# NeRdTheNed/deft4j

Hardware: AMD Instinct MI355X
Metric: input MB/s on raw-deflate optimise (mode NONE) (higher is better)
Workload: dtype u8

## Files before the change

### deft4j_amd/__init__.py

```python
import ctypes
import os

_HERE = os.path.dirname(os.path.abspath(__file__))
LIB_PATH = os.path.join(_HERE, "libdeft4g.so")

_lib = None
_ready = False


class d4g_stats(ctypes.Structure):
    _fields_ = [(n, ctypes.c_double) for n in ("ms_upload", "ms_parse", "ms_optimise", "ms_merge", "ms_write", "ms_total")] + \
               [(n, ctypes.c_int64) for n in ("n_streams", "n_blocks", "n_tokens", "bytes_in", "bytes_decoded", "bytes_out",
                                              "rounds", "kernel_launches", "search_bytes_algorithmic")] + \
               [("ms_search_kernels", ctypes.c_double), ("ms_parse_kernels", ctypes.c_double)] + \
               [(n, ctypes.c_int64) for n in ("scan_candidates", "scan_confirmed", "exact_probes", "jump_rounds")] + \
               [("ms_state_kernels", ctypes.c_double), ("state_launches", ctypes.c_int64), ("state_tokens_per_round", ctypes.c_int64),
                ("state_bytes_per_round", ctypes.c_int64), ("search_lanes", ctypes.c_int64), ("ms_checksum_kernels", ctypes.c_double),
                ("ms_lz_sort", ctypes.c_double), ("ms_lz_parse", ctypes.c_double), ("ms_lz_emit", ctypes.c_double),
                ("lz_parse_passes", ctypes.c_int64), ("lz_chunks_rerun", ctypes.c_int64), ("lz_symbols", ctypes.c_int64),
                ("ms_recompress_encode", ctypes.c_double), ("ms_recompress_encode_front", ctypes.c_double),
                ("ms_recompress_encode_search", ctypes.c_double), ("ms_recompress_reoptimise", ctypes.c_double),
                ("recompress_outputs", ctypes.c_int64), ("recompress_outputs_pruned", ctypes.c_int64),
                ("ms_zopfli_table", ctypes.c_double), ("ms_zopfli_split", ctypes.c_double), ("ms_zopfli_squeeze", ctypes.c_double),
                ("ms_zopfli_emit", ctypes.c_double), ("zopfli_blocks", ctypes.c_int64), ("zopfli_position_iterations", ctypes.c_int64),
# ... 50 lines not shown
VERIFY_OK, VERIFY_SKIPPED, VERIFY_PARSE, VERIFY_SIZE, VERIFY_LENGTH, VERIFY_BYTES = 0, 1, -1, -2, -3, -4
VERDICT_NAMES = {0: "OK", 1: "SKIPPED", -1: "PARSE", -2: "SIZE", -3: "LENGTH", -4: "BYTES"}
BLOCK_TYPE_NAMES = ("STORED", "FIXED", "DYNAMIC")

ENC_JVM, ENC_JZLIB = 0, 1
STRATEGY_DEFAULT, STRATEGY_FILTERED, STRATEGY_HUFFMAN_ONLY = 0, 1, 2
STRATEGY_RLE, STRATEGY_FIXED = 3, 4

EXPORTS = ["d4g_init", "d4g_shutdown", "d4g_last_error", "d4g_batch_create", "d4g_batch_run", "d4g_batch_stream_result",
           "d4g_batch_copy_output", "d4g_batch_copy_decoded", "d4g_batch_checksums", "d4g_batch_parse", "d4g_batch_stats", "d4g_batch_destroy", "d4g_optimise_streams",
           "d4g_size_bits_fallback", "d4g_inflate", "d4g_free", "d4g_batch_create_encode", "d4g_batch_run_encode", "d4g_deflate_streams",
           "d4g_compress", "d4g_recompress_streams", "d4g_batch_run_recompress", "d4g_batch_recompress_result", "d4g_zopfli_streams",
           "d4g_debug_zopfli_table", "d4g_debug_zopfli_code_lengths", "d4g_debug_cl_tree_lengths", "d4g_init_devices", "d4g_device_count", "d4g_set_device",
           "d4g_batch_create_on", "d4g_optimise_streams_sharded", "d4g_batch_create_encode_level", "d4g_deflate_streams_level",
           "d4g_batch_verify", "d4g_batch_verify_result", "d4g_verify_streams", "d4g_debug_batch_poke_output", "d4g_batch_block_info", "d4g_debug_verify_compare",
           "d4g_debug_device_blocks", "d4g_batch_parse_error", "d4g_diagnose_streams", "d4g_parse_reason_name",
           "d4g_find_streams", "d4g_batch_recover", "d4g_batch_copy_recovered", "d4g_recover_streams"]


def load_library(path=None):
    global _lib
    if _lib is not None and path is None:
        return _lib
    p = path or os.environ.get("D4G_LIB") or LIB_PATH
    if not os.path.exists(p):
        raise RuntimeError("libdeft4g.so is not built (%s): run `python -c 'import __graft_entry__ as g; g.build()'`; "
                           "there is no CPU fallback" % p)
    L = ctypes.CDLL(p)
    L.d4g_init.restype = ctypes.c_int
    L.d4g_init.argtypes = [ctypes.c_int]
    L.d4g_shutdown.restype = None
# ... 76 lines not shown
    L.d4g_optimise_streams_sharded.restype = ctypes.c_int
    L.d4g_optimise_streams_sharded.argtypes = L.d4g_optimise_streams.argtypes
    L.d4g_batch_verify.restype = ctypes.c_int
    L.d4g_batch_verify.argtypes = [ctypes.c_void_p]
    L.d4g_batch_verify_result.restype = ctypes.c_int
    L.d4g_batch_verify_result.argtypes = [ctypes.c_void_p, ctypes.c_size_t, ctypes.POINTER(ctypes.c_int32), ctypes.POINTER(ctypes.c_int64)]
    L.d4g_verify_streams.restype = ctypes.c_int
    L.d4g_verify_streams.argtypes = [ctypes.c_size_t, ctypes.POINTER(ctypes.c_char_p), ctypes.POINTER(ctypes.c_size_t), ctypes.POINTER(ctypes.c_char_p),
                                     ctypes.POINTER(ctypes.c_size_t), ctypes.POINTER(ctypes.c_int32), ctypes.POINTER(ctypes.c_int64)]
    L.d4g_debug_batch_poke_output.restype = ctypes.c_int
    L.d4g_debug_batch_poke_output.argtypes = [ctypes.c_void_p, ctypes.c_size_t, ctypes.c_size_t, ctypes.c_uint8]
    L.d4g_debug_verify_compare.restype = ctypes.c_int
    L.d4g_debug_verify_compare.argtypes = [ctypes.c_char_p, ctypes.c_size_t, ctypes.c_char_p, ctypes.c_size_t, ctypes.c_size_t, ctypes.POINTER(ctypes.c_int64)]
    L.d4g_debug_device_blocks.restype = ctypes.c_int
    L.d4g_debug_device_blocks.argtypes = [ctypes.POINTER(ctypes.c_int64)]
    L.d4g_batch_block_info.restype = ctypes.c_int
    L.d4g_batch_block_info.argtypes = [ctypes.c_void_p, ctypes.c_size_t, ctypes.c_int, ctypes.POINTER(d4g_block_info), ctypes.c_size_t,
                                       ctypes.POINTER(ctypes.c_size_t)]
    L.d4g_batch_parse_error.restype = ctypes.c_int
    L.d4g_batch_parse_error.argtypes = [ctypes.c_void_p, ctypes.c_size_t, ctypes.POINTER(d4g_parse_error)]
    L.d4g_diagnose_streams.restype = ctypes.c_int
    L.d4g_diagnose_streams.argtypes = [ctypes.c_size_t, ctypes.POINTER(ctypes.c_char_p), ctypes.POINTER(ctypes.c_size_t), ctypes.POINTER(d4g_parse_error)]
    L.d4g_parse_reason_name.restype = ctypes.c_char_p
    L.d4g_parse_reason_name.argtypes = [ctypes.c_int]
    L.d4g_find_streams.restype = ctypes.c_int
    L.d4g_find_streams.argtypes = [ctypes.c_size_t, ctypes.POINTER(ctypes.c_char_p), ctypes.POINTER(ctypes.c_size_t), ctypes.POINTER(d4g_find_options),
                                   ctypes.POINTER(ctypes.POINTER(d4g_found_stream)), ctypes.POINTER(ctypes.c_size_t), ctypes.POINTER(d4g_find_stats)]
    L.d4g_batch_recover.restype = ctypes.c_int
    L.d4g_batch_recover.argtypes = [ctypes.c_void_p]
    L.d4g_batch_copy_recovered.restype = ctypes.c_int
# ... 548 lines not shown
```

### deft4j_amd/csrc/d4g_arch.h

```cpp
#pragma once
#include <stdint.h>

#ifndef D4G_HOSTSIM
#include <hip/hip_runtime.h>
#endif

#if defined(D4G_PROFILE_OPS) && defined(D4G_HOSTSIM)
#error "D4G_PROFILE_OPS counts GPU clock cycles: the emulator build has no clock"
#endif

#define D4G_DEV __device__ __forceinline__

#if defined(D4G_HOSTSIM) && !defined(D4G_SIM_WAVE_HEAP)
#define D4G_SERIAL_TREES
#endif

#ifdef D4G_HOSTSIM
#define D4G_SIM_LOG(...) fprintf(stderr, __VA_ARGS__)
#else
#define D4G_SIM_LOG(...) ((void)0)
#endif

#define D4G_BASE_PRIO 1
#ifdef D4G_HOSTSIM
// ... 37 lines not shown
#endif
}

D4G_DEV int wave_sum_i32(int v) {
#ifdef D4G_HOSTSIM
    for (int m = 32; m >= 1; m >>= 1) v = (int)((unsigned)v + (unsigned)__shfl_xor(v, m));
    return v;
#else
    v += __builtin_amdgcn_update_dpp(0, v, 0x111, 0xf, 0xf, false);
    v += __builtin_amdgcn_update_dpp(0, v, 0x112, 0xf, 0xf, false);
    v += __builtin_amdgcn_update_dpp(0, v, 0x114, 0xf, 0xf, false);
    v += __builtin_amdgcn_update_dpp(0, v, 0x118, 0xf, 0xf, false);
    v += __builtin_amdgcn_update_dpp(0, v, 0x142, 0xa, 0xf, false);
    v += __builtin_amdgcn_update_dpp(0, v, 0x143, 0xc, 0xf, false);
    return __builtin_amdgcn_readlane(v, 63);
#endif
}

D4G_DEV uint32_t wave_min_u32(uint32_t v) {
#ifdef D4G_HOSTSIM
    for (int m = 32; m >= 1; m >>= 1) { const uint32_t o = __shfl_xor(v, m); v = o < v ? o : v; }
    return v;
#else
    int x = (int)v;
    auto step = [&](int o) { x = (int)((uint32_t)o < (uint32_t)x ? (uint32_t)o : (uint32_t)x); };
    step(__builtin_amdgcn_update_dpp(-1, x, 0x111, 0xf, 0xf, false));
    step(__builtin_amdgcn_update_dpp(-1, x, 0x112, 0xf, 0xf, false));
    step(__builtin_amdgcn_update_dpp(-1, x, 0x114, 0xf, 0xf, false));
    step(__builtin_amdgcn_update_dpp(-1, x, 0x118, 0xf, 0xf, false));
    step(__builtin_amdgcn_update_dpp(-1, x, 0x142, 0xa, 0xf, false));
// ... 95 lines not shown
```

### deft4j_amd/csrc/d4g_host.h

```cpp
#pragma once
#include <algorithm>
#include <chrono>
#include <cstring>
#include <map>
#include <memory>
#include <atomic>
#include <vector>

#include "d4g_ops.h"
#include "d4g_fused.h"
#include "d4g_parse.h"
#include "d4g_rt.h"
#include "d4g_write.h"
#include "d4g_knobs.h"
#include "d4g_program.h"
#include "../../include/deft4g.h"

namespace d4g {

#define D4G_SEG_TARGET_BYTES 8192
#define D4G_SEG_MAX_BYTES (1LL << 20)
#define D4G_SEG_MAX_TOKENS (1LL << 16)
static inline int seg_threads() {
#ifdef D4G_HOSTSIM
    return parse_threads();
#else
    return 1024;
#endif
}

static inline double now_ms() {
    return std::chrono::duration<double, std::milli>(std::chrono::steady_clock::now().time_since_epoch()).count();
}

struct HBlock {
    int type = 0;
    int gpu = -1;
    int homeGpu = -1;
    int ordinal = 0;
    i64 tokStart = 0, tokCount = 0, uStart = 0, uLen = 0;
    i64 refStart = 0, refCount = 0;
    i64 size = 0;
// ... 188 lines not shown
```

### deft4j_amd/csrc/d4g_host_parse.h

```cpp
#pragma once

namespace d4g {

inline void Batch::create(size_t n, const uint8_t* const* in, const size_t* len, bool fromDevice) {
    memset(&stats, 0, sizeof(stats));
    double t0 = now_ms();
    streams.resize(n);
    i64 off = 0;
    for (size_t i = 0; i < n; i++) {
        streams[i].inOff = off;
        streams[i].inLen = (i64)len[i];
        off += ((i64)len[i] + 15) & ~15LL;
        off += 16;
        stats.bytes_in += (i64)len[i];
    }
    i64 total = off + D4G_INCH + 64;
    dIn.alloc_zero((size_t)total);
    for (size_t i = 0; i < n; i++) {
        if (fromDevice) rt_d2d(dIn + streams[i].inOff, in[i], len[i]);
        else rt_h2d(dIn + streams[i].inOff, in[i], len[i]);
    }
    rt_sync();
    stats.n_streams = (i64)n;
    stats.ms_upload = now_ms() - t0;
// ... 485 lines not shown
            R.maxSlots = std::max(R.maxSlots, (i64)(segs.size() - first) - 1);
            for (size_t q = first; q < segs.size(); q++)
                for (i64 o = 0; o < segs[q].uLen; o += D4G_SUB_CHUNK)
                    R.chunks.push_back({si, segs[q].win, segs[q].uStart + o, std::min<i64>(D4G_SUB_CHUNK, segs[q].uLen - o)});
        }
        i = j;
    }
    return R;
}
inline void Batch::copy_block_local(const std::vector<D4GTokRange>& allRanges, const CopyRoute& R, int32_t* dBad, RtScratch& tmp) {
    D4GTokRange* dAll = tmp.upload(allRanges);
    D4GSegment* dSegs = tmp.upload(R.segs);
    uint16_t* dSym = tmp.alloc<uint16_t>((size_t)uTotal, 64);
    const size_t slots = R.slotOrd.size();
    uint16_t* dTailA = slots ? tmp.alloc<uint16_t>(slots * D4G_WIN) : nullptr;
    RT_LAUNCH(k_seg_symbols, R.segs.size(), seg_threads(), dStreams, dSegs, dAll, dTok, dU, dSym, dTailA, dBad);
    stats.kernel_launches++;
    stats.copy_segments += (i64)R.segs.size();
    if (R.maxSlots > 1) {
        int32_t* dOrd = tmp.upload(R.slotOrd);
        uint16_t* dTailB = tmp.alloc<uint16_t>(slots * D4G_WIN);
        const int GC = 4;
        for (i64 d = 1; d < R.maxSlots; d <<= 1) {
            RT_LAUNCH(k_seg_compose, slots * GC, 256, dOrd, dTailA, dTailB, (int)d, GC);
            std::swap(dTailA, dTailB);
            stats.kernel_launches++;
            stats.copy_rounds++;
        }
    }
    if (!R.chunks.empty()) {
        D4GSubChunk* dChunks = tmp.upload(R.chunks);
// ... 78 lines not shown
        }
        bool done = false;
        for (int k = 0; k < JB; k++) {
            stats.jump_rounds++;
            if (ch[k] < stopNum) { done = true; break; }
        }
        if (done) break;
    }
    RT_LAUNCH(k_resolve_streams, n * (size_t)G, 256, dStreamsD, dSrc, dU, G);
    stats.kernel_launches++;
}
inline void Batch::block_bins(const std::vector<int32_t>& realBlocks, bool needSlots, RtScratch& tmp) {
    if (!needSlots || realBlocks.empty()) return;
    int32_t* dReal = tmp.upload(realBlocks);
    D4GCtx c = make_ctx(engine().progDyn, 0);
    RT_LAUNCH(k_block_bins, realBlocks.size() * D4G_BINS_SPLIT, 256, c, dReal);
    stats.kernel_launches++;
}

}
```

### deft4j_amd/csrc/d4g_host_write.h

```cpp
#pragma once

namespace d4g {

inline void Batch::phase_write() {
    std::vector<D4GWriteJob> jobs;
    i64 words = 0;
    for (HStream& s : streams) {
        s.outWordBase = words;
        if (s.status != 0) continue;
        i64 pos = 0;
        for (size_t k = 0; k < s.blocks.size(); k++) {
            const HBlock& b = s.blocks[k];
            D4GWriteJob j;
            memset(&j, 0, sizeof(j));
            j.blk = b.gpu;
            j.type = b.type;
            j.isFinal = k + 1 == s.blocks.size();
            j.bitStart = words * 32 + pos;
            j.uAbs = s.uBase + b.uStart;
            j.uLen = b.uLen;
            jobs.push_back(j);
            pos += 3;
            pos += b.size_at(pos);
        }
// ... 73 lines not shown
    phase_write();
    double t4 = now_ms();
    stats.ms_parse = t1 - t0;
    stats.ms_optimise = t2 - t1b;
    stats.ms_merge = t3 - t2;
    stats.ms_write = t4 - t3;
    stats.ms_total = (t1 - t0) + (t4 - t1b);
    stats.ms_search_kernels = msSearch;
    stats.ms_parse_kernels = msParseKernels;
    stats.search_bytes_algorithmic = stats.bytes_in + stats.bytes_decoded + stats.bytes_out;
    release_scratch();
}
inline void Batch::release_scratch() {
    rt_sync_all();
    dTok.reset(); dRefs.reset(); dTokRef.reset();
    dBinStat.reset(); dBinMask.reset();
    dHsMemo.reset(); dRcMemo.reset(); dPassMemo.reset();
    dBlocks.reset(); dStates.reset(); dMasks.reset();
    dKeys.reset(); dActive.reset(); dResults.reset();
    dReady.reset(); dHeads.reset();
}

enum { VERIFY_OK = 0, VERIFY_SKIPPED = 1, VERIFY_PARSE = -1, VERIFY_SIZE = -2, VERIFY_LENGTH = -3, VERIFY_BYTES = -4 };
struct VerifyItem {
    const uint8_t* bytes = nullptr;
    size_t len = 0;
    const uint8_t* want = nullptr;
    i64 wantLen = 0;
    i64 wantBits = -1;
    int verdict = VERIFY_SKIPPED;
    i64 first = -1;
// ... 63 lines not shown
```

### deft4j_amd/csrc/d4g_knobs.h

```cpp
#pragma once
#include <algorithm>
#include <cstdlib>
#include <cstring>
#include <stdexcept>

#include "d4g_ops.h"
#include "d4g_fused.h"
#include "d4g_rt.h"

namespace d4g {

static inline const char* knob_now(const char* name) { return getenv(name); }
static inline int knob_now(const char* name, int def) { const char* t = getenv(name); return t ? atoi(t) : def; }
static inline long long knob_now_ll(const char* name, long long def) { const char* t = getenv(name); return t ? atoll(t) : def; }
#define KNOB_ONCE(name, def) ([] { static const int v = knob_now(name, def); return v; }())
static inline bool knob_is_zero(const char* t) { return t && t[0] == '0'; }

static inline bool exec_fused() { const char* t = knob_now("D4G_EXEC"); return !t || !strcmp(t, "fused"); }
static inline int exec_persistent(int nActive = 0) {
    const char* t = knob_now("D4G_EXEC");
    const int mode = !t ? 2 : !strcmp(t, "levels") ? 0 : !strcmp(t, "persistent") ? 1 : 2;
    const int maxBlocks = knob_now("D4G_PERSIST_MAX_BLOCKS", 128);
#ifdef D4G_HOSTSIM
    return mode == 0 ? 0 : 1;
// ... 56 lines not shown
#endif
    return v == 128 || v == 256 || v == 512 ? v : 64;
}
enum { D4G_COPY_AUTO = 0, D4G_COPY_DOUBLING = 1, D4G_COPY_BLOCKS = 2 };
static inline int copy_mode() {
    const char* t = knob_now("D4G_COPY");
    if (!t || !strcmp(t, "auto")) return D4G_COPY_AUTO;
    if (!strcmp(t, "doubling")) return D4G_COPY_DOUBLING;
    if (!strcmp(t, "blocks")) return D4G_COPY_BLOCKS;
    throw std::runtime_error("D4G_COPY must be doubling, blocks or auto");
}
static inline int jump_stop_pct() { return KNOB_ONCE("D4G_JUMP_STOP_PCT", 50); }
static inline int jump_tile_reps() { return KNOB_ONCE("D4G_JUMP_TILE_REPS", 6); }
static inline int jump_threads() { return KNOB_ONCE("D4G_JUMP_THREADS", 1024); }
static inline int jump_lds_kb() { return KNOB_ONCE("D4G_JUMP_LDS_KB", 70); }

static inline bool verify_switch() { const char* v = knob_now("D4G_VERIFY"); return v && v[0] && !(v[0] == '0' && !v[1]); }
static inline void pool_max_bytes(size_t* bytes) { if (const char* t = knob_now("D4G_POOL_MAX_MB")) *bytes = (size_t)atoll(t) << 20; }
static inline long long group_blocks() { return knob_now("D4G_GROUP_BLOCKS", 12000); }
static inline bool zf_table_scan() { const char* t = knob_now("D4G_ZF_TABLE"); return t && !strcmp(t, "scan"); }
static inline int zf_pool_words() { const char* t = knob_now("D4G_ZF_POOL_WORDS"); return t ? std::max(64, atoi(t)) : 0; }

static inline bool debug_rounds() { return knob_now("D4G_DEBUG_ROUNDS") != nullptr; }
static inline bool debug_jump() { return knob_now("D4G_DEBUG_JUMP") != nullptr; }
static inline int debug_program() { const char* t = knob_now("D4G_DEBUG_PROGRAM"); return !t ? 0 : atoi(t) >= 2 ? 2 : 1; }
static inline int debug_zopfli() { return knob_now("D4G_DEBUG_ZOPFLI", 0); }

}
```

### deft4j_amd/csrc/d4g_ops.h

```cpp
#pragma once
#include "d4g_device.h"

#ifdef D4G_PROFILE_OPS
__device__ unsigned long long d4g_dbg_pass[4];
__device__ unsigned long long d4g_dbg_hdr[4];
#endif

#ifndef D4G_HSMEMO_SLOTS
#define D4G_HSMEMO_SLOTS 64
#endif
struct D4GHsMemo {
    unsigned long long tag;
    unsigned long long check;
    int32_t state;
    int32_t hdr;
    int32_t lane;
    int32_t nLit;
    int32_t n, pad;
    uint32_t key[(D4G_NLIT + D4G_NDIST) / 4];
};

#ifndef D4G_RCMEMO_SLOTS
#define D4G_RCMEMO_SLOTS 128
#endif
// ... 379 lines not shown
        atomicAdd(&d4g_dbg_pass[3], (unsigned long long)nRef);
    }
#endif
    if (mine) {
        for (int i = threadIdx.x; i < D4G_HIST; i += blockDim.x) d4g_st_agent((uint32_t*)&mine->delta[i], (uint32_t)((int)S->hist[i] - histBefore[i]));
        if (threadIdx.x == 0) {
            d4g_st_agent((uint64_t*)&mine->saved, (uint64_t)saved);
            d4g_st_agent((uint64_t*)&mine->check, (uint64_t)h2);
        }
        d4g_drain_stores();
        __syncthreads();
        if (threadIdx.x == 0) d4g_st_agent(&mine->state, 2);
    }
}

#define D4G_BINS_SPLIT 4
__global__ void __launch_bounds__(256) k_block_bins(D4GCtx c, const int32_t* blockList) {
    __shared__ uint32_t T[D4G_NBINS * D4G_BINSTRIDE];
    const D4GBlock b = c.blocks[blockList[blockIdx.x / D4G_BINS_SPLIT]];
    const int part = blockIdx.x % D4G_BINS_SPLIT;
    if (b.binStat < 0) return;
    for (int i = threadIdx.x; i < D4G_NBINS * D4G_BINSTRIDE; i += blockDim.x) T[i] = 0;
    __syncthreads();
    const uint4* rf = c.refs + b.refStart;
    const uint8_t* Ub = c.U + b.uBase;
    uint64_t* bm = c.binMask + b.binMask;
    const int lane = threadIdx.x & 63;
    const int nRef = (int)b.refCount, nWords = (int)b.maskWords;
    for (int r0 = part * (int)blockDim.x; r0 < nWords * 64; r0 += D4G_BINS_SPLIT * (int)blockDim.x) {
        int r = r0 + threadIdx.x;
        uint4 rv = r < nRef ? rf[r] : make_uint4(0u, 0u, 0u, 0u);
        int len = ref_len(rv.x);
        int bin = ref_lsym(rv.x) - 257;
        if (len > 0) {
            const uint32_t* uw = (const uint32_t*)Ub + (rv.y >> 2);
            const int sh = (int)(rv.y & 3u) * 8;
            uint32_t w0 = uw[0], w1 = uw[1], w2 = uw[2];
            c.refs[b.refStart + r].z = d4g_alignbit(w1, w0, sh);
            c.refs[b.refStart + r].w = d4g_alignbit(w2, w1, sh);
            uint32_t* row = T + bin * D4G_BINSTRIDE;
            atomicAdd(&row[D4G_BIN_DIST + ref_dsym(rv.x)], 1u);
            atomicAdd(&row[D4G_BIN_COUNT], 1u);
            atomicAdd(&row[D4G_BIN_EBITS], (unsigned)ref_ebits(rv.x));
            for_bytes(Ub + rv.y, len, [&](int by) { atomicAdd(&row[by], 1u); return true; });
        }
        unsigned long long todo = d4g_ballot(len > 0);
        while (todo) {
            int src = __ffsll((long long)todo) - 1;
            int bsel = __shfl(bin, src);
            unsigned long long same = d4g_ballot(len > 0 && bin == bsel);
            if (lane == src) bm[(long long)bsel * nWords + (r >> 6)] = same;
            todo &= ~same;
        }
    }
    __syncthreads();
    uint32_t* g = c.binStat + b.binStat;
    for (int i = threadIdx.x; i < D4G_NBINS * D4G_BINSTRIDE; i += blockDim.x)
        if (T[i]) atomicAdd(&g[i], T[i]);
}

D4G_DEV int d4g_ref_lit_total(const uint32_t* Uw, const uint16_t* lc, uint32_t off, int len) {
    D4GLitWalk lw;
    lw_start(lw, Uw, off, len);
    while (lw.rem > 0) lw_step(lw, Uw, lc);
    return lw.total;
}
// ... 1248 lines not shown
```

### deft4j_amd/csrc/d4g_parse.h

```cpp
#pragma once
#include <type_traits>

#include "d4g_device.h"

struct D4GStreamDesc {
    const uint8_t* data;
    long long len;
    long long uBase;
    long long uLen;
};

struct D4GProbeIn {
    int32_t stream;
    int32_t strict;
    long long bitPos;
};
struct D4GProbeOut {
    int32_t status;
    int32_t type;
    int32_t bfinal;
    int32_t eofHit;
    long long endBit;
    long long nTok, uLen, sizeBits;
    long long needHist;
// ... 1079 lines not shown
    int32_t tail;
    int32_t win;
    int32_t pad;
    long long uStart, uLen;
};
#define D4G_SUB_CHUNK 65536
struct D4GSubChunk { int32_t stream, win; long long first, count; };
struct D4GSegLds {
    uint16_t ring[D4G_SEG_RING];
    uint32_t pos[D4G_SEG_GROUP_TOKENS + 1];
    uint32_t a[D4G_SEG_GROUP_TOKENS + 1];
    int n;
    int anyPtr[3];
};

__global__ void __launch_bounds__(1024) k_seg_symbols(const D4GStreamDesc* streams, const D4GSegment* segs, const D4GTokRange* ranges,
                                                                      const uint2* tok, const uint8_t* U, uint16_t* sym, uint16_t* tails,
                                                                      int32_t* badDist) {
    __shared__ D4GSegLds L;
    const int tid = threadIdx.x, NL = blockDim.x;
    const D4GSegment sg = segs[blockIdx.x];
    const D4GStreamDesc sd = streams[sg.stream];
    uint16_t* out = sym + sd.uBase + sg.uStart;
    const uint32_t segStart = (uint32_t)sg.uStart;
    for (int i = tid; i < D4G_WIN; i += NL) L.ring[i] = (uint16_t)(D4G_SYM_MARK | (uint32_t)i);
    if (tid == 0) { L.n = D4G_SEG_GROUP_TOKENS; L.anyPtr[0] = 0; L.anyPtr[1] = 0; L.anyPtr[2] = 0; }
    __syncthreads();
    int rr = 0;
    bool bad = false;
    for (int r = 0; r < sg.rangeCount; r++) {
        const D4GTokRange rg = ranges[sg.rangeFirst + r];
        const uint32_t b0 = (uint32_t)(rg.uStart - sg.uStart), bLen = (uint32_t)rg.uLen;
        if (rg.stored) {
            const uint8_t* u = U + sd.uBase + rg.uStart;
            for (uint32_t k = tid; k < bLen; k += NL) {
                const uint16_t v = u[k];
                if (bLen - k <= D4G_WIN) L.ring[(b0 + k + D4G_WIN) % D4G_SEG_RING] = v;
                out[b0 + k] = v;
            }
            __syncthreads();
            continue;
        }
        const uint2* tk = tok + rg.tokStart;
        long long t0 = 0;
        uint32_t gs = b0;
        uint2 pre = make_uint2(0u, 0u);
        if (tid < rg.tokCount) pre = tk[tid];
        while (t0 < rg.tokCount) {
            const long long left = rg.tokCount - t0;
            const int m = left < D4G_SEG_GROUP_TOKENS ? (int)left : D4G_SEG_GROUP_TOKENS, m1 = left < D4G_SEG_GROUP_TOKENS + 1 ? (int)left : D4G_SEG_GROUP_TOKENS + 1;
            for (int i = tid; i <= D4G_SEG_GROUP_TOKENS; i += NL) {
                if (i >= m1) { L.pos[i] = 0xffffffffu; continue; }
                const uint2 t = i == tid ? pre : tk[t0 + i];
                const uint32_t p = t.y - segStart;
                const int dist = tok_dist(t.x), val = tok_val(t.x);
                const uint32_t len = dist ? (uint32_t)val : (val < 256 ? 1u : 0u);
                L.pos[i] = p;
                L.a[i] = t.x;
                if (i < m && p + len - gs > D4G_SEG_GROUP_BYTES) atomicMin(&L.n, i);
            }
            __syncthreads();
            const int n = L.n < m ? L.n : m;
            const uint32_t ge = n < m1 ? L.pos[n] : b0 + bLen;
            if (t0 + n + tid < rg.tokCount) pre = tk[t0 + n + tid];
            constexpr int K = 4;
            for (uint32_t base = gs + tid; base < ge; base += K * NL) {
                uint32_t j[K], e[K];
                int lo[K];
#pragma unroll
                for (int k = 0; k < K; k++) { j[k] = base + k * NL; lo[k] = 0; }
#pragma unroll
                for (int st = (D4G_SEG_GROUP_TOKENS + 1) / 2; st > 0; st >>= 1) {
#pragma unroll
                    for (int k = 0; k < K; k++)
                        if (L.pos[lo[k] + st] <= j[k]) lo[k] += st;
                }
#pragma unroll
                for (int k = 0; k < K; k++) {
                    const bool in = j[k] < ge;
                    const uint32_t a = L.a[in ? lo[k] : 0];
                    const uint32_t dist = in ? (uint32_t)tok_dist(a) : 0u;
                    const uint32_t back = L.ring[(j[k] + D4G_WIN - dist) % D4G_SEG_RING];
                    if (!dist) e[k] = a & 0xffu;
                    else if (dist > segStart + j[k]) { e[k] = 0; bad = true; }
                    else if (j[k] - gs >= dist) e[k] = D4G_SYM_PTR | (j[k] - dist - gs);
                    else e[k] = back;
                }
#pragma unroll
                for (int k = 0; k < K; k++)
                    if (j[k] < ge) L.ring[(j[k] + D4G_WIN) % D4G_SEG_RING] = (uint16_t)e[k];
            }
            __syncthreads();
            if (tid == 0) L.n = D4G_SEG_GROUP_TOKENS;
            for (;;) {
                bool mine = false;
                for (uint32_t base = gs + tid; base < ge; base += K * NL) {
                    uint32_t e[K], e2[K];
#pragma unroll
                    for (int k = 0; k < K; k++) e[k] = base + k * NL < ge ? L.ring[(base + k * NL + D4G_WIN) % D4G_SEG_RING] : 0u;
#pragma unroll
                    for (int k = 0; k < K; k++) e2[k] = L.ring[(gs + (e[k] & 0x3fffu) + D4G_WIN) % D4G_SEG_RING];
#pragma unroll
                    for (int k = 0; k < K; k++)
                        if ((e[k] & 0xc000u) == D4G_SYM_PTR) {
                            L.ring[(base + k * NL + D4G_WIN) % D4G_SEG_RING] = (uint16_t)e2[k];
                            mine |= (e2[k] & 0xc000u) == D4G_SYM_PTR;
                        }
                }
                if (mine) L.anyPtr[rr % 3] = 1;
                if (tid == 0) L.anyPtr[(rr + 1) % 3] = 0;
                __syncthreads();
                const int any = L.anyPtr[rr % 3];
                rr++;
                if (!any) break;
            }
            for (uint32_t j = gs + tid; j < ge; j += NL) out[j] = L.ring[(j + D4G_WIN) % D4G_SEG_RING];
            gs = ge;
            t0 += n;
        }
        __syncthreads();
    }
    if (bad) badDist[sg.stream] = 1;
    if (sg.tail >= 0) {
        __syncthreads();
        uint16_t* t = tails + (long long)sg.tail * D4G_WIN;
        const uint32_t q0 = (uint32_t)sg.uLen;
        for (int i = tid; i < D4G_WIN; i += NL) t[i] = L.ring[(q0 + (uint32_t)i) % D4G_SEG_RING];
    }
}

__global__ void __launch_bounds__(256) k_seg_compose(const int32_t* slotOrd, const uint16_t* in, uint16_t* out, int d, int G) {
    const long long slot = blockIdx.x / G;
    const bool look = slotOrd[slot] >= d;
    const uint4* a = (const uint4*)(in + slot * D4G_WIN);
    uint4* o = (uint4*)(out + slot * D4G_WIN);
    const uint16_t* prev = in + (slot - (look ? d : 0)) * D4G_WIN;
    auto via = [&](uint32_t w) D4G_LAMBDA_INLINE {
        uint32_t lo = w & 0xffffu, hi = w >> 16;
        if (lo & D4G_SYM_MARK) lo = prev[lo & 0x7fffu];
        if (hi & D4G_SYM_MARK) hi = prev[hi & 0x7fffu];
        return lo | (hi << 16);
    };
    for (int i = (blockIdx.x % G) * blockDim.x + threadIdx.x; i < D4G_WIN / 8; i += G * blockDim.x) {
        uint4 v = a[i];
// ... 40 lines not shown
```

### deft4j_amd/csrc/libdeft4g.hip

```cpp
#include <functional>
#include <mutex>
#include <thread>

#include "d4g_host.h"
#include "d4g_lz77_host.h"
#include "d4g_zopfli_host.h"
#include "d4g_host_find.h"

using namespace d4g;

struct d4g_batch {
    int ctx = 0;
    Batch impl;
    std::unique_ptr<LzFront> lz;
    std::unique_ptr<Batch> reopt;
    std::vector<int> reoptIndex;
    std::vector<char> graft;
    std::vector<int64_t> recompSaved;
    bool verified = false;
    std::vector<int32_t> verdict;
    std::vector<int64_t> firstMismatch;
    std::vector<std::vector<Batch::PBlock>> finalBlocks;
    const HStream& final_stream(size_t i, const Batch** owner) const {
        if (i < graft.size() && graft[i]) { *owner = reopt.get(); return reopt->streams[reoptIndex[i]]; }
// ... 1320 lines not shown
                d4g_pack_kinds(v, r, flags, [&](int sym, int run, int, int cnt) { b[sym * 160 + run] += cnt; }, [&](int cnt) { b[v * 160] += cnt; });
                for (int i = 0; i < 19 * 160; i++) bad += a[i] != b[i];
            }
    return bad;
}
#endif

int d4g_debug_device_blocks(int64_t* live) {
    if (!live) return fail(D4G_ERR_ARG, "null argument");
    return api(nullptr, [&] {
        *live = (int64_t)rt_live_blocks();
        return D4G_OK;
    });
}

int d4g_debug_fused_stats(long long* out64) {
    return api(nullptr, [&] {
        engine().init();
        rt_sync_all();
        rt_d2h(out64, engine().dOpStats, 64 * 8);
        rt_memset(engine().dOpStats, 0, 64 * 8);
        rt_sync();
        return D4G_OK;
    });
}

#ifdef D4G_PROFILE_OPS
int d4g_debug_set_experiment(long long mode) {
    return api(nullptr, [&] {
        rt_h2d(engine().dOpStats + 63, &mode, 8);
// ... 18 lines not shown
```

### include/deft4g.h

```cpp
#ifndef DEFT4G_H
#define DEFT4G_H

#include <stddef.h>
#include <stdint.h>

#ifdef __cplusplus
extern "C" {
#endif

#define D4G_OK 0
#define D4G_ERR_NODEVICE (-1)
#define D4G_ERR_ARG (-2)
#define D4G_ERR_RUNTIME (-3)

#define D4G_STREAM_CHANGED 0
#define D4G_STREAM_UNCHANGED 1
#define D4G_STREAM_PARSE_ERROR (-1)

typedef struct d4g_batch d4g_batch;

typedef struct d4g_stats {
    double ms_upload, ms_parse, ms_optimise, ms_merge, ms_write, ms_total;
    int64_t n_streams, n_blocks, n_tokens, bytes_in, bytes_decoded, bytes_out;
    int64_t rounds, kernel_launches;
// ... 86 lines not shown
#define D4G_VERIFY_OK 0
#define D4G_VERIFY_SKIPPED 1
#define D4G_VERIFY_PARSE (-1)
#define D4G_VERIFY_SIZE (-2)
#define D4G_VERIFY_LENGTH (-3)
#define D4G_VERIFY_BYTES (-4)
int d4g_batch_verify(d4g_batch* b);
int d4g_batch_verify_result(d4g_batch* b, size_t i, int32_t* verdict, int64_t* first_mismatch);
int d4g_verify_streams(size_t n, const uint8_t* const* a, const size_t* a_len, const uint8_t* const* b, const size_t* b_len,
                       int32_t* verdict, int64_t* first_mismatch);
int d4g_debug_batch_poke_output(d4g_batch* b, size_t i, size_t byte_offset, uint8_t xor_mask);
int d4g_debug_verify_compare(const uint8_t* x, size_t x_skew, const uint8_t* y, size_t y_skew, size_t len, int64_t* first);

int d4g_debug_device_blocks(int64_t* live);

typedef struct d4g_block_info { int32_t type, bfinal; int64_t bit_pos, size_bits, header_bits, tokens, decoded_len; } d4g_block_info;
int d4g_batch_block_info(d4g_batch* b, size_t i, int which , d4g_block_info* out, size_t cap,
                         size_t* n_blocks);

#define D4G_PARSE_OK 0
#define D4G_PARSE_EOF 1
#define D4G_PARSE_BLOCK_TYPE 2
#define D4G_PARSE_STORED_LENGTHS 3
#define D4G_PARSE_CODE_LENGTHS 4
#define D4G_PARSE_LITLEN_SYMBOL 5
#define D4G_PARSE_DIST_SYMBOL 6
#define D4G_PARSE_DISTANCE_TOO_FAR 7
typedef struct d4g_parse_error {
    int32_t reason, block;
    int64_t block_bit_pos, bit_pos;
// ... 45 lines not shown
```

Measured before the change: 15660.

## Rebalance block-bins byte histogram across wave lanes with adaptive split

Reworks k_block_bins so each wave computes a prefix scan of reference lengths and spreads the per-byte histogram work evenly across lanes, either by walking a dense covering range word by word or by splitting the total byte count among lanes. Previously each lane serially walked its own reference's bytes, which left lanes idle when match lengths were uneven. It also raises the block to 512 threads and picks the split per block from the block count, aiming to fill the GPU when there are few blocks. Adds debug-only timing stamps for the segment kernel and a bin-table readback API, both gated by environment variables.

After: 16250, median of 6. +3.7%, better.

```diff
diff --git a/deft4j_amd/__init__.py b/deft4j_amd/__init__.py
--- a/deft4j_amd/__init__.py
+++ b/deft4j_amd/__init__.py
@@ -88,7 +88,7 @@
            "d4g_debug_zopfli_table", "d4g_debug_zopfli_code_lengths", "d4g_debug_cl_tree_lengths", "d4g_init_devices", "d4g_device_count", "d4g_set_device",
            "d4g_batch_create_on", "d4g_optimise_streams_sharded", "d4g_batch_create_encode_level", "d4g_deflate_streams_level",
            "d4g_batch_verify", "d4g_batch_verify_result", "d4g_verify_streams", "d4g_debug_batch_poke_output", "d4g_batch_block_info", "d4g_debug_verify_compare",
-           "d4g_debug_device_blocks", "d4g_batch_parse_error", "d4g_diagnose_streams", "d4g_parse_reason_name",
+           "d4g_debug_device_blocks", "d4g_debug_batch_bins", "d4g_batch_parse_error", "d4g_diagnose_streams", "d4g_parse_reason_name",
            "d4g_find_streams", "d4g_batch_recover", "d4g_batch_copy_recovered", "d4g_recover_streams"]
 
 
@@ -195,6 +195,8 @@
     L.d4g_debug_verify_compare.argtypes = [ctypes.c_char_p, ctypes.c_size_t, ctypes.c_char_p, ctypes.c_size_t, ctypes.c_size_t, ctypes.POINTER(ctypes.c_int64)]
     L.d4g_debug_device_blocks.restype = ctypes.c_int
     L.d4g_debug_device_blocks.argtypes = [ctypes.POINTER(ctypes.c_int64)]
+    L.d4g_debug_batch_bins.restype = ctypes.c_int
+    L.d4g_debug_batch_bins.argtypes = [ctypes.c_void_p, ctypes.c_size_t, ctypes.c_void_p, ctypes.c_void_p, ctypes.POINTER(ctypes.c_size_t)]
     L.d4g_batch_block_info.restype = ctypes.c_int
     L.d4g_batch_block_info.argtypes = [ctypes.c_void_p, ctypes.c_size_t, ctypes.c_int, ctypes.POINTER(d4g_block_info), ctypes.c_size_t,
                                        ctypes.POINTER(ctypes.c_size_t)]
diff --git a/deft4j_amd/csrc/d4g_arch.h b/deft4j_amd/csrc/d4g_arch.h
--- a/deft4j_amd/csrc/d4g_arch.h
+++ b/deft4j_amd/csrc/d4g_arch.h
@@ -75,6 +75,22 @@
     v += __builtin_amdgcn_update_dpp(0, v, 0x142, 0xa, 0xf, false);
     v += __builtin_amdgcn_update_dpp(0, v, 0x143, 0xc, 0xf, false);
     return __builtin_amdgcn_readlane(v, 63);
+#endif
+}
+
+D4G_DEV int wave_scan_i32(int v) {
+#ifdef D4G_HOSTSIM
+    const int lane = (int)(threadIdx.x & 63);
+    for (int d = 1; d < 64; d <<= 1) { const int o = __shfl_up(v, d); if (lane >= d) v += o; }
+    return v;
+#else
+    v += __builtin_amdgcn_update_dpp(0, v, 0x111, 0xf, 0xf, false);
+    v += __builtin_amdgcn_update_dpp(0, v, 0x112, 0xf, 0xf, false);
+    v += __builtin_amdgcn_update_dpp(0, v, 0x114, 0xf, 0xf, false);
+    v += __builtin_amdgcn_update_dpp(0, v, 0x118, 0xf, 0xf, false);
+    v += __builtin_amdgcn_update_dpp(0, v, 0x142, 0xa, 0xf, false);
+    v += __builtin_amdgcn_update_dpp(0, v, 0x143, 0xc, 0xf, false);
+    return v;
 #endif
 }
 
diff --git a/deft4j_amd/csrc/d4g_host.h b/deft4j_amd/csrc/d4g_host.h
--- a/deft4j_amd/csrc/d4g_host.h
+++ b/deft4j_amd/csrc/d4g_host.h
@@ -26,6 +26,13 @@
     return parse_threads();
 #else
     return 1024;
+#endif
+}
+static inline int bins_threads() {
+#ifdef D4G_HOSTSIM
+    return 256;
+#else
+    return D4G_BINS_THREADS;
 #endif
 }
 
diff --git a/deft4j_amd/csrc/d4g_host_parse.h b/deft4j_amd/csrc/d4g_host_parse.h
--- a/deft4j_amd/csrc/d4g_host_parse.h
+++ b/deft4j_amd/csrc/d4g_host_parse.h
@@ -523,7 +523,17 @@
     uint16_t* dSym = tmp.alloc<uint16_t>((size_t)uTotal, 64);
     const size_t slots = R.slotOrd.size();
     uint16_t* dTailA = slots ? tmp.alloc<uint16_t>(slots * D4G_WIN) : nullptr;
-    RT_LAUNCH(k_seg_symbols, R.segs.size(), seg_threads(), dStreams, dSegs, dAll, dTok, dU, dSym, dTailA, dBad);
+    if (seg_stamps()) {
+        unsigned long long* dSt = tmp.alloc_zero<unsigned long long>(D4G_SEG_STAMP_SLOTS);
+        RT_LAUNCH(k_seg_symbols_stamped, R.segs.size(), seg_threads(), dStreams, dSegs, dAll, dTok, dU, dSym, dTailA, dBad, dSt);
+        unsigned long long st[D4G_SEG_STAMP_SLOTS];
+        rt_d2h(st, dSt, sizeof(st));
+        fprintf(stderr, "seg stamps: wgs %llu groups %llu rounds %llu | cycles: staging %llu search %llu writeout %llu tail %llu other %llu | whole %llu longest %llu | round r cycles/groups:",
+                st[9], st[7], st[8], st[0], st[1], st[2], st[3], st[4], st[5], st[6]);
+        for (int q = 0; q < 8; q++) fprintf(stderr, " %llu/%llu", st[16 + q], st[24 + q]);
+        fprintf(stderr, "\n");
+    } else
+        RT_LAUNCH(k_seg_symbols, R.segs.size(), seg_threads(), dStreams, dSegs, dAll, dTok, dU, dSym, dTailA, dBad);
     stats.kernel_launches++;
     stats.copy_segments += (i64)R.segs.size();
     if (R.maxSlots > 1) {
@@ -632,7 +642,8 @@
     if (!needSlots || realBlocks.empty()) return;
     int32_t* dReal = tmp.upload(realBlocks);
     D4GCtx c = make_ctx(engine().progDyn, 0);
-    RT_LAUNCH(k_block_bins, realBlocks.size() * D4G_BINS_SPLIT, 256, c, dReal);
+    const int split = d4g_bins_split(realBlocks.size());
+    RT_LAUNCH(k_block_bins, realBlocks.size() * (size_t)split, bins_threads(), c, dReal, split);
     stats.kernel_launches++;
 }
 
diff --git a/deft4j_amd/csrc/d4g_host_write.h b/deft4j_amd/csrc/d4g_host_write.h
--- a/deft4j_amd/csrc/d4g_host_write.h
+++ b/deft4j_amd/csrc/d4g_host_write.h
@@ -111,7 +111,7 @@
 inline void Batch::release_scratch() {
     rt_sync_all();
     dTok.reset(); dRefs.reset(); dTokRef.reset();
-    dBinStat.reset(); dBinMask.reset();
+    if (!keep_bins()) { dBinStat.reset(); dBinMask.reset(); }
     dHsMemo.reset(); dRcMemo.reset(); dPassMemo.reset();
     dBlocks.reset(); dStates.reset(); dMasks.reset();
     dKeys.reset(); dActive.reset(); dResults.reset();
diff --git a/deft4j_amd/csrc/d4g_knobs.h b/deft4j_amd/csrc/d4g_knobs.h
--- a/deft4j_amd/csrc/d4g_knobs.h
+++ b/deft4j_amd/csrc/d4g_knobs.h
@@ -94,6 +94,8 @@
 static inline int jump_tile_reps() { return KNOB_ONCE("D4G_JUMP_TILE_REPS", 6); }
 static inline int jump_threads() { return KNOB_ONCE("D4G_JUMP_THREADS", 1024); }
 static inline int jump_lds_kb() { return KNOB_ONCE("D4G_JUMP_LDS_KB", 70); }
+static inline bool seg_stamps() { return knob_now("D4G_SEG_STAMPS") != nullptr; }
+static inline bool keep_bins() { return knob_now("D4G_KEEP_BINS") != nullptr; }
 
 static inline bool verify_switch() { const char* v = knob_now("D4G_VERIFY"); return v && v[0] && !(v[0] == '0' && !v[1]); }
 static inline void pool_max_bytes(size_t* bytes) { if (const char* t = knob_now("D4G_POOL_MAX_MB")) *bytes = (size_t)atoll(t) << 20; }
diff --git a/deft4j_amd/csrc/d4g_ops.h b/deft4j_amd/csrc/d4g_ops.h
--- a/deft4j_amd/csrc/d4g_ops.h
+++ b/deft4j_amd/csrc/d4g_ops.h
@@ -417,26 +417,43 @@
     }
 }
 
-#define D4G_BINS_SPLIT 4
-__global__ void __launch_bounds__(256) k_block_bins(D4GCtx c, const int32_t* blockList) {
+#define D4G_BINS_THREADS 512
+#define D4G_BINS_SLOTS 768
+#define D4G_BINS_MAXSPLIT 16
+#define D4G_BINS_DENSE 4
+inline int d4g_bins_split(size_t nBlocks) {
+    const size_t s = nBlocks ? D4G_BINS_SLOTS / nBlocks : 1;
+    return (int)(s < 1 ? 1 : s > D4G_BINS_MAXSPLIT ? D4G_BINS_MAXSPLIT : s);
+}
+struct D4GBinsWave {
+    uint32_t start[65];
+    uint16_t end[64];
+    uint16_t len[64];
+    uint16_t row[64];
+};
+__global__ void __launch_bounds__(D4G_BINS_THREADS) k_block_bins(D4GCtx c, const int32_t* blockList, int split) {
     __shared__ uint32_t T[D4G_NBINS * D4G_BINSTRIDE];
-    const D4GBlock b = c.blocks[blockList[blockIdx.x / D4G_BINS_SPLIT]];
-    const int part = blockIdx.x % D4G_BINS_SPLIT;
+    __shared__ D4GBinsWave W[D4G_BINS_THREADS / 64];
+    const D4GBlock b = c.blocks[blockList[blockIdx.x / split]];
+    const int part = blockIdx.x % split;
     if (b.binStat < 0) return;
     for (int i = threadIdx.x; i < D4G_NBINS * D4G_BINSTRIDE; i += blockDim.x) T[i] = 0;
     __syncthreads();
     const uint4* rf = c.refs + b.refStart;
     const uint8_t* Ub = c.U + b.uBase;
+    const uint32_t* Uw = (const uint32_t*)Ub;
     uint64_t* bm = c.binMask + b.binMask;
-    const int lane = threadIdx.x & 63;
+    const int lane = threadIdx.x & 63, wave = threadIdx.x >> 6, nw = blockDim.x >> 6;
     const int nRef = (int)b.refCount, nWords = (int)b.maskWords;
-    for (int r0 = part * (int)blockDim.x; r0 < nWords * 64; r0 += D4G_BINS_SPLIT * (int)blockDim.x) {
-        int r = r0 + threadIdx.x;
+    D4GBinsWave& R = W[wave];
+    if (lane == 0) R.start[64] = 0xffffffffu;
+    for (int w = part * nw + wave; w < nWords; w += split * nw) {
+        const int r = w * 64 + lane;
         uint4 rv = r < nRef ? rf[r] : make_uint4(0u, 0u, 0u, 0u);
         int len = ref_len(rv.x);
         int bin = ref_lsym(rv.x) - 257;
         if (len > 0) {
-            const uint32_t* uw = (const uint32_t*)Ub + (rv.y >> 2);
+            const uint32_t* uw = Uw + (rv.y >> 2);
             const int sh = (int)(rv.y & 3u) * 8;
             uint32_t w0 = uw[0], w1 = uw[1], w2 = uw[2];
             c.refs[b.refStart + r].z = d4g_alignbit(w1, w0, sh);
@@ -445,14 +462,66 @@
             atomicAdd(&row[D4G_BIN_DIST + ref_dsym(rv.x)], 1u);
             atomicAdd(&row[D4G_BIN_COUNT], 1u);
             atomicAdd(&row[D4G_BIN_EBITS], (unsigned)ref_ebits(rv.x));
-            for_bytes(Ub + rv.y, len, [&](int by) { atomicAdd(&row[by], 1u); return true; });
         }
         unsigned long long todo = d4g_ballot(len > 0);
+        const int nv = __popcll(todo);
+        const int mine = wave_scan_i32(len);
+        R.start[lane] = len > 0 ? rv.y : 0xffffffffu;
+        R.end[lane] = (uint16_t)mine;
+        R.len[lane] = (uint16_t)len;
+        R.row[lane] = (uint16_t)(bin * D4G_BINSTRIDE);
+        d4g_wave_sync();
+        if (nv) {
+            const int total = (int)R.end[63];
+            const uint32_t s0 = R.start[0] & ~3u, sEnd = R.start[nv - 1] + R.len[nv - 1];
+            if (sEnd - s0 <= (uint32_t)(D4G_BINS_DENSE * total)) {
+                uint32_t p = s0 + 4u * (uint32_t)lane;
+                uint32_t wa = p < sEnd ? Uw[p >> 2] : 0u, wb = p + 256u < sEnd ? Uw[(p + 256u) >> 2] : 0u;
+                for (; p < sEnd; p += 256u) {
+                    uint32_t word = wa;
+                    wa = wb;
+                    wb = p + 512u < sEnd ? Uw[(p + 512u) >> 2] : 0u;
+                    int i = 0;
+                    for (int s = 32; s; s >>= 1)
+                        if (R.start[i + s] <= p) i += s;
+                    uint32_t st = R.start[i], en = st + R.len[i], nx = R.start[i + 1];
+                    uint32_t* row = T + R.row[i];
+#pragma unroll
+                    for (uint32_t q = p; q < p + 4u; q++, word >>= 8) {
+                        if (q >= nx) {
+                            i++;
+                            st = nx; en = st + R.len[i]; nx = R.start[i + 1];
+                            row = T + R.row[i];
+                        }
+                        if (q >= st && q < en) atomicAdd(&row[word & 0xffu], 1u);
+                    }
+                }
+            } else {
+                const int per = (total + 63) >> 6;
+                int k = lane * per;
+                const int k1 = k + per < total ? k + per : total;
+                if (k < k1) {
+                    int i = 0;
+                    for (int s = 32; s; s >>= 1)
+                        if ((int)R.end[i + s - 1] <= k) i += s;
+                    int start = i ? (int)R.end[i - 1] : 0;
+                    while (k < k1) {
+                        const int e = (int)R.end[i];
+                        const int n = (e < k1 ? e : k1) - k;
+                        uint32_t* row = T + R.row[i];
+                        for_bytes(Ub + R.start[i] + (k - start), n, [&](int by) { atomicAdd(&row[by], 1u); return true; });
+                        k += n;
+                        start = e;
+                        i++;
+                    }
+                }
+            }
+        }
         while (todo) {
             int src = __ffsll((long long)todo) - 1;
             int bsel = __shfl(bin, src);
             unsigned long long same = d4g_ballot(len > 0 && bin == bsel);
-            if (lane == src) bm[(long long)bsel * nWords + (r >> 6)] = same;
+            if (lane == src) bm[(long long)bsel * nWords + w] = same;
             todo &= ~same;
         }
     }
diff --git a/deft4j_amd/csrc/d4g_parse.h b/deft4j_amd/csrc/d4g_parse.h
--- a/deft4j_amd/csrc/d4g_parse.h
+++ b/deft4j_amd/csrc/d4g_parse.h
@@ -1117,120 +1117,21 @@
     int anyPtr[3];
 };
 
+#define D4G_SEG_STAMP_SLOTS 32
+#define D4G_SEG_ST 0
 __global__ void __launch_bounds__(1024) k_seg_symbols(const D4GStreamDesc* streams, const D4GSegment* segs, const D4GTokRange* ranges,
                                                                       const uint2* tok, const uint8_t* U, uint16_t* sym, uint16_t* tails,
                                                                       int32_t* badDist) {
-    __shared__ D4GSegLds L;
-    const int tid = threadIdx.x, NL = blockDim.x;
-    const D4GSegment sg = segs[blockIdx.x];
-    const D4GStreamDesc sd = streams[sg.stream];
-    uint16_t* out = sym + sd.uBase + sg.uStart;
-    const uint32_t segStart = (uint32_t)sg.uStart;
-    for (int i = tid; i < D4G_WIN; i += NL) L.ring[i] = (uint16_t)(D4G_SYM_MARK | (uint32_t)i);
-    if (tid == 0) { L.n = D4G_SEG_GROUP_TOKENS; L.anyPtr[0] = 0; L.anyPtr[1] = 0; L.anyPtr[2] = 0; }
-    __syncthreads();
-    int rr = 0;
-    bool bad = false;
-    for (int r = 0; r < sg.rangeCount; r++) {
-        const D4GTokRange rg = ranges[sg.rangeFirst + r];
-        const uint32_t b0 = (uint32_t)(rg.uStart - sg.uStart), bLen = (uint32_t)rg.uLen;
-        if (rg.stored) {
-            const uint8_t* u = U + sd.uBase + rg.uStart;
-            for (uint32_t k = tid; k < bLen; k += NL) {
-                const uint16_t v = u[k];
-                if (bLen - k <= D4G_WIN) L.ring[(b0 + k + D4G_WIN) % D4G_SEG_RING] = v;
-                out[b0 + k] = v;
-            }
-            __syncthreads();
-            continue;
-        }
-        const uint2* tk = tok + rg.tokStart;
-        long long t0 = 0;
-        uint32_t gs = b0;
-        uint2 pre = make_uint2(0u, 0u);
-        if (tid < rg.tokCount) pre = tk[tid];
-        while (t0 < rg.tokCount) {
-            const long long left = rg.tokCount - t0;
-            const int m = left < D4G_SEG_GROUP_TOKENS ? (int)left : D4G_SEG_GROUP_TOKENS, m1 = left < D4G_SEG_GROUP_TOKENS + 1 ? (int)left : D4G_SEG_GROUP_TOKENS + 1;
-            for (int i = tid; i <= D4G_SEG_GROUP_TOKENS; i += NL) {
-                if (i >= m1) { L.pos[i] = 0xffffffffu; continue; }
-                const uint2 t = i == tid ? pre : tk[t0 + i];
-                const uint32_t p = t.y - segStart;
-                const int dist = tok_dist(t.x), val = tok_val(t.x);
-                const uint32_t len = dist ? (uint32_t)val : (val < 256 ? 1u : 0u);
-                L.pos[i] = p;
-                L.a[i] = t.x;
-                if (i < m && p + len - gs > D4G_SEG_GROUP_BYTES) atomicMin(&L.n, i);
-            }
-            __syncthreads();
-            const int n = L.n < m ? L.n : m;
-            const uint32_t ge = n < m1 ? L.pos[n] : b0 + bLen;
-            if (t0 + n + tid < rg.tokCount) pre = tk[t0 + n + tid];
-            constexpr int K = 4;
-            for (uint32_t base = gs + tid; base < ge; base += K * NL) {
-                uint32_t j[K], e[K];
-                int lo[K];
-#pragma unroll
-                for (int k = 0; k < K; k++) { j[k] = base + k * NL; lo[k] = 0; }
-#pragma unroll
-                for (int st = (D4G_SEG_GROUP_TOKENS + 1) / 2; st > 0; st >>= 1) {
-#pragma unroll
-                    for (int k = 0; k < K; k++)
-                        if (L.pos[lo[k] + st] <= j[k]) lo[k] += st;
-                }
-#pragma unroll
-                for (int k = 0; k < K; k++) {
-                    const bool in = j[k] < ge;
-                    const uint32_t a = L.a[in ? lo[k] : 0];
-                    const uint32_t dist = in ? (uint32_t)tok_dist(a) : 0u;
-                    const uint32_t back = L.ring[(j[k] + D4G_WIN - dist) % D4G_SEG_RING];
-                    if (!dist) e[k] = a & 0xffu;
-                    else if (dist > segStart + j[k]) { e[k] = 0; bad = true; }
-                    else if (j[k] - gs >= dist) e[k] = D4G_SYM_PTR | (j[k] - dist - gs);
-                    else e[k] = back;
-                }
-#pragma unroll
-                for (int k = 0; k < K; k++)
-                    if (j[k] < ge) L.ring[(j[k] + D4G_WIN) % D4G_SEG_RING] = (uint16_t)e[k];
-            }
-            __syncthreads();
-            if (tid == 0) L.n = D4G_SEG_GROUP_TOKENS;
-            for (;;) {
-                bool mine = false;
-                for (uint32_t base = gs + tid; base < ge; base += K * NL) {
-                    uint32_t e[K], e2[K];
-#pragma unroll
-                    for (int k = 0; k < K; k++) e[k] = base + k * NL < ge ? L.ring[(base + k * NL + D4G_WIN) % D4G_SEG_RING] : 0u;
-#pragma unroll
-                    for (int k = 0; k < K; k++) e2[k] = L.ring[(gs + (e[k] & 0x3fffu) + D4G_WIN) % D4G_SEG_RING];
-#pragma unroll
-                    for (int k = 0; k < K; k++)
-                        if ((e[k] & 0xc000u) == D4G_SYM_PTR) {
-                            L.ring[(base + k * NL + D4G_WIN) % D4G_SEG_RING] = (uint16_t)e2[k];
-                            mine |= (e2[k] & 0xc000u) == D4G_SYM_PTR;
-                        }
-                }
-                if (mine) L.anyPtr[rr % 3] = 1;
-                if (tid == 0) L.anyPtr[(rr + 1) % 3] = 0;
-                __syncthreads();
-                const int any = L.anyPtr[rr % 3];
-                rr++;
-                if (!any) break;
-            }
-            for (uint32_t j = gs + tid; j < ge; j += NL) out[j] = L.ring[(j + D4G_WIN) % D4G_SEG_RING];
-            gs = ge;
-            t0 += n;
-        }
-        __syncthreads();
-    }
-    if (bad) badDist[sg.stream] = 1;
-    if (sg.tail >= 0) {
-        __syncthreads();
-        uint16_t* t = tails + (long long)sg.tail * D4G_WIN;
-        const uint32_t q0 = (uint32_t)sg.uLen;
-        for (int i = tid; i < D4G_WIN; i += NL) t[i] = L.ring[(q0 + (uint32_t)i) % D4G_SEG_RING];
-    }
-}
+#include "d4g_seg_symbols.inc"
+}
+#undef D4G_SEG_ST
+#define D4G_SEG_ST 1
+__global__ void __launch_bounds__(1024) k_seg_symbols_stamped(const D4GStreamDesc* streams, const D4GSegment* segs, const D4GTokRange* ranges,
+                                                                              const uint2* tok, const uint8_t* U, uint16_t* sym, uint16_t* tails,
+                                                                              int32_t* badDist, unsigned long long* stamps) {
+#include "d4g_seg_symbols.inc"
+}
+#undef D4G_SEG_ST
 
 __global__ void __launch_bounds__(256) k_seg_compose(const int32_t* slotOrd, const uint16_t* in, uint16_t* out, int d, int G) {
     const long long slot = blockIdx.x / G;
diff --git a/deft4j_amd/csrc/d4g_seg_symbols.inc b/deft4j_amd/csrc/d4g_seg_symbols.inc
--- /dev/null
+++ b/deft4j_amd/csrc/d4g_seg_symbols.inc
@@ -0,0 +1,156 @@
+    __shared__ D4GSegLds L;
+    const int tid = threadIdx.x, NL = blockDim.x;
+#if D4G_SEG_ST
+    uint32_t acc[5] = {0u, 0u, 0u, 0u, 0u}, accR[8] = {0u, 0u, 0u, 0u, 0u, 0u, 0u, 0u}, cntR[8] = {0u, 0u, 0u, 0u, 0u, 0u, 0u, 0u}, nGroups = 0;
+    long long tBegin = 0, tPrev = 0;
+    auto lap = [&]() -> uint32_t { const long long t = d4g_clock_drained(); const uint32_t d = (uint32_t)(t - tPrev); tPrev = t; return d; };
+    if (tid == 0) tBegin = tPrev = d4g_clock_drained();
+#endif
+    const D4GSegment sg = segs[blockIdx.x];
+    const D4GStreamDesc sd = streams[sg.stream];
+    uint16_t* out = sym + sd.uBase + sg.uStart;
+    const uint32_t segStart = (uint32_t)sg.uStart;
+    for (int i = tid; i < D4G_WIN; i += NL) L.ring[i] = (uint16_t)(D4G_SYM_MARK | (uint32_t)i);
+    if (tid == 0) { L.n = D4G_SEG_GROUP_TOKENS; L.anyPtr[0] = 0; L.anyPtr[1] = 0; L.anyPtr[2] = 0; }
+    __syncthreads();
+#if D4G_SEG_ST
+    if (tid == 0) acc[4] += lap();
+#endif
+    int rr = 0;
+    bool bad = false;
+    for (int r = 0; r < sg.rangeCount; r++) {
+        const D4GTokRange rg = ranges[sg.rangeFirst + r];
+        const uint32_t b0 = (uint32_t)(rg.uStart - sg.uStart), bLen = (uint32_t)rg.uLen;
+        if (rg.stored) {
+            const uint8_t* u = U + sd.uBase + rg.uStart;
+            for (uint32_t k = tid; k < bLen; k += NL) {
+                const uint16_t v = u[k];
+                if (bLen - k <= D4G_WIN) L.ring[(b0 + k + D4G_WIN) % D4G_SEG_RING] = v;
+                out[b0 + k] = v;
+            }
+            __syncthreads();
+#if D4G_SEG_ST
+            if (tid == 0) acc[4] += lap();
+#endif
+            continue;
+        }
+        const uint2* tk = tok + rg.tokStart;
+        long long t0 = 0;
+        uint32_t gs = b0;
+        uint2 pre = make_uint2(0u, 0u);
+        if (tid < rg.tokCount) pre = tk[tid];
+        while (t0 < rg.tokCount) {
+            const long long left = rg.tokCount - t0;
+            const int m = left < D4G_SEG_GROUP_TOKENS ? (int)left : D4G_SEG_GROUP_TOKENS, m1 = left < D4G_SEG_GROUP_TOKENS + 1 ? (int)left : D4G_SEG_GROUP_TOKENS + 1;
+            for (int i = tid; i <= D4G_SEG_GROUP_TOKENS; i += NL) {
+                if (i >= m1) { L.pos[i] = 0xffffffffu; continue; }
+                const uint2 t = i == tid ? pre : tk[t0 + i];
+                const uint32_t p = t.y - segStart;
+                const int dist = tok_dist(t.x), val = tok_val(t.x);
+                const uint32_t len = dist ? (uint32_t)val : (val < 256 ? 1u : 0u);
+                L.pos[i] = p;
+                L.a[i] = t.x;
+                if (i < m && p + len - gs > D4G_SEG_GROUP_BYTES) atomicMin(&L.n, i);
+            }
+            __syncthreads();
+#if D4G_SEG_ST
+            if (tid == 0) { acc[0] += lap(); nGroups++; }
+#endif
+            const int n = L.n < m ? L.n : m;
+            const uint32_t ge = n < m1 ? L.pos[n] : b0 + bLen;
+            if (t0 + n + tid < rg.tokCount) pre = tk[t0 + n + tid];
+            constexpr int K = 4;
+            for (uint32_t base = gs + tid; base < ge; base += K * NL) {
+                uint32_t j[K], e[K];
+                int lo[K];
+#pragma unroll
+                for (int k = 0; k < K; k++) { j[k] = base + k * NL; lo[k] = 0; }
+#pragma unroll
+                for (int st = (D4G_SEG_GROUP_TOKENS + 1) / 2; st > 0; st >>= 1) {
+#pragma unroll
+                    for (int k = 0; k < K; k++)
+                        if (L.pos[lo[k] + st] <= j[k]) lo[k] += st;
+                }
+#pragma unroll
+                for (int k = 0; k < K; k++) {
+                    const bool in = j[k] < ge;
+                    const uint32_t a = L.a[in ? lo[k] : 0];
+                    const uint32_t dist = in ? (uint32_t)tok_dist(a) : 0u;
+                    const uint32_t back = L.ring[(j[k] + D4G_WIN - dist) % D4G_SEG_RING];
+                    if (!dist) e[k] = a & 0xffu;
+                    else if (dist > segStart + j[k]) { e[k] = 0; bad = true; }
+                    else if (j[k] - gs >= dist) e[k] = D4G_SYM_PTR | (j[k] - dist - gs);
+                    else e[k] = back;
+                }
+#pragma unroll
+                for (int k = 0; k < K; k++)
+                    if (j[k] < ge) L.ring[(j[k] + D4G_WIN) % D4G_SEG_RING] = (uint16_t)e[k];
+            }
+            __syncthreads();
+#if D4G_SEG_ST
+            if (tid == 0) acc[1] += lap();
+            const int rr0 = rr;
+#endif
+            if (tid == 0) L.n = D4G_SEG_GROUP_TOKENS;
+            for (;;) {
+                bool mine = false;
+                for (uint32_t base = gs + tid; base < ge; base += K * NL) {
+                    uint32_t e[K], e2[K];
+#pragma unroll
+                    for (int k = 0; k < K; k++) e[k] = base + k * NL < ge ? L.ring[(base + k * NL + D4G_WIN) % D4G_SEG_RING] : 0u;
+#pragma unroll
+                    for (int k = 0; k < K; k++) e2[k] = L.ring[(gs + (e[k] & 0x3fffu) + D4G_WIN) % D4G_SEG_RING];
+#pragma unroll
+                    for (int k = 0; k < K; k++)
+                        if ((e[k] & 0xc000u) == D4G_SYM_PTR) {
+                            L.ring[(base + k * NL + D4G_WIN) % D4G_SEG_RING] = (uint16_t)e2[k];
+                            mine |= (e2[k] & 0xc000u) == D4G_SYM_PTR;
+                        }
+                }
+                if (mine) L.anyPtr[rr % 3] = 1;
+                if (tid == 0) L.anyPtr[(rr + 1) % 3] = 0;
+                __syncthreads();
+#if D4G_SEG_ST
+                if (tid == 0) {
+                    const uint32_t d = lap();
+                    const int ri = rr - rr0 < 7 ? rr - rr0 : 7;
+#pragma unroll
+                    for (int q = 0; q < 8; q++) { accR[q] += q == ri ? d : 0u; cntR[q] += q == ri ? 1u : 0u; }
+                }
+#endif
+                const int any = L.anyPtr[rr % 3];
+                rr++;
+                if (!any) break;
+            }
+            for (uint32_t j = gs + tid; j < ge; j += NL) out[j] = L.ring[(j + D4G_WIN) % D4G_SEG_RING];
+#if D4G_SEG_ST
+            if (tid == 0) acc[2] += lap();
+#endif
+            gs = ge;
+            t0 += n;
+        }
+        __syncthreads();
+#if D4G_SEG_ST
+        if (tid == 0) acc[4] += lap();
+#endif
+    }
+    if (bad) badDist[sg.stream] = 1;
+    if (sg.tail >= 0) {
+        __syncthreads();
+        uint16_t* t = tails + (long long)sg.tail * D4G_WIN;
+        const uint32_t q0 = (uint32_t)sg.uLen;
+        for (int i = tid; i < D4G_WIN; i += NL) t[i] = L.ring[(q0 + (uint32_t)i) % D4G_SEG_RING];
+    }
+#if D4G_SEG_ST
+    if (tid == 0) {
+        acc[3] += lap();
+        const unsigned long long whole = (unsigned long long)(tPrev - tBegin);
+        for (int q = 0; q < 5; q++) atomicAdd(&stamps[q], (unsigned long long)acc[q]);
+        atomicAdd(&stamps[5], whole);
+        atomicMax(&stamps[6], whole);
+        atomicAdd(&stamps[7], (unsigned long long)nGroups);
+        atomicAdd(&stamps[8], (unsigned long long)rr);
+        atomicAdd(&stamps[9], 1ull);
+        for (int q = 0; q < 8; q++) { atomicAdd(&stamps[16 + q], (unsigned long long)accR[q]); atomicAdd(&stamps[24 + q], (unsigned long long)cntR[q]); }
+    }
+#endif
diff --git a/deft4j_amd/csrc/libdeft4g.hip b/deft4j_amd/csrc/libdeft4g.hip
--- a/deft4j_amd/csrc/libdeft4g.hip
+++ b/deft4j_amd/csrc/libdeft4g.hip
@@ -1358,6 +1358,23 @@
     });
 }
 
+static_assert(D4G_DEBUG_BINS_ROWS == D4G_NBINS && D4G_DEBUG_BINS_STRIDE == D4G_BINSTRIDE, "deft4g.h describes the bin table");
+int d4g_debug_batch_bins(d4g_batch* b, size_t block, uint32_t* table, uint64_t* masks, size_t* mask_words) {
+    return api(b, [&] {
+        if (!b || !table || !mask_words) return fail(D4G_ERR_ARG, "null argument");
+        const Batch& B = b->impl;
+        if (!B.dBinStat || !B.dBinMask) return fail(D4G_ERR_ARG, "the batch has no bin tables (not run, or released: D4G_KEEP_BINS)");
+        if (block >= B.hBlocks.size() || B.hBlocks[block].binStat < 0) return fail(D4G_ERR_ARG, "bad block index");
+        const D4GBlock& hb = B.hBlocks[block];
+        rt_sync_all();
+        rt_d2h(table, B.dBinStat + hb.binStat, (size_t)D4G_NBINS * D4G_BINSTRIDE * 4);
+        const size_t room = *mask_words, words = (size_t)D4G_NBINS * (size_t)hb.maskWords;
+        *mask_words = (size_t)hb.maskWords;
+        if (masks && words && words <= room) rt_d2h(masks, B.dBinMask + hb.binMask, words * 8);
+        return D4G_OK;
+    });
+}
+
 int d4g_debug_fused_stats(long long* out64) {
     return api(nullptr, [&] {
         engine().init();
diff --git a/include/deft4g.h b/include/deft4g.h
--- a/include/deft4g.h
+++ b/include/deft4g.h
@@ -124,6 +124,10 @@
 
 int d4g_debug_device_blocks(int64_t* live);
 
+#define D4G_DEBUG_BINS_ROWS 29
+#define D4G_DEBUG_BINS_STRIDE 320
+int d4g_debug_batch_bins(d4g_batch* b, size_t block, uint32_t* table, uint64_t* masks, size_t* mask_words);
+
 typedef struct d4g_block_info { int32_t type, bfinal; int64_t bit_pos, size_bits, header_bits, tokens, decoded_len; } d4g_block_info;
 int d4g_batch_block_info(d4g_batch* b, size_t i, int which , d4g_block_info* out, size_t cap,
                          size_t* n_blocks);
```
